# zhvng/open-musiclm

Measured on NVIDIA H100. Metric: coarse-stage training tokens/sec (positions fed to the transformer per optimiser step / step time), higher is better.
Workload: dtype bf16 (fp16 operands for the forward GEMMs on LayerNorm outputs x weights; fp32 accumulate)

## Files before the change

open-musiclm_b200/csrc/gemm_tc.cu:

```cuda
#include "common.cuh"
#include "ptx.cuh"
#include "../../include/omlm_b200.h"
#include <stdlib.h>
#include <algorithm>

namespace omlm {

constexpr int BM = 128;
constexpr int BK = 64;
constexpr int kGemmThreads = 384;

struct EpiParams {
  void* out;
  const float* addend;
  long ldo;
  long ldadd;
  float alpha;
  int out_f32;
  int atomic;
  long split_stride;
  int vec_ok;
  int row_split;
  int row_valid;
  int n_valid;
  const __nv_bfloat16* rs_hn;
  long rs_ldhn;
  const float* rs_gamma;
  const uint8_t* rs_keep;
  float2* rs_part;
  float rs_keep_scale;
  int rs_parts;
};

__device__ __forceinline__ float bf16lo(uint32_t v) { return __uint_as_float(v << 16); }
__device__ __forceinline__ float bf16hi(uint32_t v) { return __uint_as_float(v & 0xffff0000u); }

template <int BN>
struct GemmSmem {
  static constexpr int kABytes = BM * BK * 2;
  static constexpr int kBBytes = BN * BK * 2;
  static constexpr int kStageBytes = kABytes + kBBytes;
  static constexpr int kMaxStages = 8;
};

template <int BN, int A_MN, int B_MN, bool F16, bool RS = false>
__global__ void __launch_bounds__(kGemmThreads, 1)
gemm_bf16_kernel(const __grid_constant__ CUtensorMap tmA, const __grid_constant__ CUtensorMap tmB,
                 const EpiParams ep, const int M, const int N, const int K, const int splits, const int kStages) {
  using S = GemmSmem<BN>;
  extern __shared__ uint8_t smem_raw[];
  uint8_t* smem = smem_raw + ((1024u - (smem_u32(smem_raw) & 1023u)) & 1023u);
  uint64_t* full_bar = reinterpret_cast<uint64_t*>(smem + kStages * S::kStageBytes);
  uint64_t* empty_bar = full_bar + S::kMaxStages;

  const int wg = threadIdx.x >> 7;
  const int lane = threadIdx.x & 31;

  const int m_tiles = (M + BM - 1) / BM;
  const int n_tiles = (N + BN - 1) / BN;
  const int kb_total = (K + BK - 1) / BK;
  const int kb_per_split = (kb_total + splits - 1) / splits;
  const int tiles_total = m_tiles * n_tiles;
  const int work_total = tiles_total * splits;

  if (threadIdx.x == 0) {
    tma_prefetch_desc(&tmA);
    tma_prefetch_desc(&tmB);
    for (int i = 0; i < kStages; ++i) {
      mbar_init(&full_bar[i], 1);
      mbar_init(&empty_bar[i], 2);
    }
    fence_barrier_init();
  }
  __syncthreads();

  if (wg == 0) {
    asm volatile("setmaxnreg.dec.sync.aligned.u32 40;");
    if (threadIdx.x == 0) {
      int stage = 0;
      uint32_t phase = 0;
      for (int w = blockIdx.x; w < work_total; w += gridDim.x) {
        const int split = w / tiles_total;
        const int tile = w - split * tiles_total;
        const int n_blk = tile % n_tiles, m_blk = tile / n_tiles;
        const int kb0 = split * kb_per_split;
        const int kb1 = min(kb_total, kb0 + kb_per_split);
        for (int kb = kb0; kb < kb1; ++kb) {
          mbar_wait(&empty_bar[stage], phase ^ 1);
          uint8_t* sa = smem + stage * S::kStageBytes;
          uint8_t* sb = sa + S::kABytes;
          mbar_expect_tx(&full_bar[stage], S::kStageBytes);
          if (A_MN == 0) {
            tma_load_2d(sa, &tmA, &full_bar[stage], kb * BK, m_blk * BM);
          } else {
#pragma unroll
            for (int c = 0; c < BM / 64; ++c)
              tma_load_2d(sa + c * 8192, &tmA, &full_bar[stage], m_blk * BM + c * 64, kb * BK);
          }
          if (B_MN == 0) {
            tma_load_2d(sb, &tmB, &full_bar[stage], kb * BK, n_blk * BN);
          } else {
#pragma unroll
            for (int c = 0; c < BN / 64; ++c)
              tma_load_2d(sb + c * 8192, &tmB, &full_bar[stage], n_blk * BN + c * 64, kb * BK);
          }
          if (++stage == kStages) { stage = 0; phase ^= 1; }
        }
      }
    }
    return;
  }

  asm volatile("setmaxnreg.inc.sync.aligned.u32 232;");
  const int cw = wg - 1;
  const int wq = (threadIdx.x >> 5) & 3;
  const int qr = lane >> 2, qc = lane & 3;
  const bool leader = (threadIdx.x & 127) == 0;
  int stage = 0;
  uint32_t phase = 0;
  for (int w = blockIdx.x; w < work_total; w += gridDim.x) {
    const int split = w / tiles_total;
    const int tile = w - split * tiles_total;
    const int n_blk = tile % n_tiles, m_blk = tile / n_tiles;
    const int kb0 = split * kb_per_split;
    const int kb1 = min(kb_total, kb0 + kb_per_split);
    float acc[BN / 2];
#pragma unroll
    for (int i = 0; i < BN / 2; ++i) acc[i] = 0.f;
    int prev = -1;
    for (int kb = kb0; kb < kb1; ++kb) {
      mbar_wait(&full_bar[stage], phase);
      const uint32_t sa = smem_u32(smem + stage * S::kStageBytes) + cw * 8192;
      const uint32_t sb = smem_u32(smem + stage * S::kStageBytes + S::kABytes);
      wgmma_fence();
#pragma unroll
      for (int k = 0; k < BK / 16; ++k) {
        const uint64_t ad = A_MN ? make_smem_desc(sa + k * 2048, 8192, 1024) : make_smem_desc(sa + k * 32, 16, 1024);
        const uint64_t bd = B_MN ? make_smem_desc(sb + k * 2048, 8192, 1024) : make_smem_desc(sb + k * 32, 16, 1024);
        const uint32_t accum = (kb > kb0 || k > 0) ? 1u : 0u;
        Wgmma<BN, F16>::template ss<A_MN, B_MN>(acc, ad, bd, accum);
      }
      wgmma_commit();
      wgmma_wait<1>();
      if (prev >= 0 && leader) mbar_arrive(&empty_bar[prev]);
      prev = stage;
      if (++stage == kStages) { stage = 0; phase ^= 1; }
    }
    wgmma_wait<0>();
    wgmma_reg_fence(acc);
    if (prev >= 0 && leader) mbar_arrive(&empty_bar[prev]);

    int row_in[2];
    long orow[2], arow[2];
    bool row_ok[2];
#pragma unroll
    for (int hr = 0; hr < 2; ++hr) {
      int row = m_blk * BM + cw * 64 + wq * 16 + qr + hr * 8;
      row_in[hr] = row;
      row_ok[hr] = row < M;
      if (ep.row_split > 0) {
        const int half = row / ep.row_split, r = row - half * ep.row_split;
        row_ok[hr] = row_ok[hr] && r < ep.row_valid;
        row = half * ep.row_valid + r;
      } else if (ep.row_split < 0) {
        const int w256 = row & 255, ch = ((row >> 8) << 7) + (w256 & 127);
        row_ok[hr] = row_ok[hr] && ch < ep.row_valid;
        row = (w256 >> 7) * ep.row_valid + ch;
      }
      orow[hr] = static_cast<long>(row) * ep.ldo;
      arow[hr] = static_cast<long>(row) * ep.ldadd;
    }
    constexpr int kEpiBatch = RS ? 4 : 8;
    float rs1[2][2] = {{0.f, 0.f}, {0.f, 0.f}}, rs2[2][2] = {{0.f, 0.f}, {0.f, 0.f}};
#pragma unroll
    for (int i0 = 0; i0 < BN / 8; i0 += kEpiBatch) {
      float2 add[2][kEpiBatch], gam[kEpiBatch];
      uint32_t hv[2][kEpiBatch], keep[2][kEpiBatch];
#pragma unroll
      for (int j = 0; j < kEpiBatch; ++j) {
        const int col = n_blk * BN + 8 * (i0 + j) + 2 * qc;
        const bool c0_ok = col < ep.n_valid, c1_ok = col + 1 < ep.n_valid;
        if constexpr (RS) gam[j] = c0_ok ? __ldg(reinterpret_cast<const float2*>(ep.rs_gamma + col)) : make_float2(0.f, 0.f);
#pragma unroll
        for (int hr = 0; hr < 2; ++hr) {
          add[hr][j] = make_float2(0.f, 0.f);
          hv[hr][j] = 0u;
          keep[hr][j] = 0xffu;
          if (!row_ok[hr] || !c0_ok) continue;
          if (!RS && ep.addend != nullptr) {
            const float* ap = ep.addend + arow[hr] + col;
            if (c1_ok && ep.vec_ok) add[hr][j] = *reinterpret_cast<const float2*>(ap);
            else { add[hr][j].x = ap[0]; if (c1_ok) add[hr][j].y = ap[1]; }
          }
          if constexpr (RS) {
            hv[hr][j] = *reinterpret_cast<const uint32_t*>(ep.rs_hn + static_cast<long>(row_in[hr]) * ep.rs_ldhn + col);
            if (ep.rs_keep != nullptr) keep[hr][j] = ep.rs_keep[static_cast<long>(row_in[hr]) * (N >> 3) + (col >> 3)];
          }
        }
      }
#pragma unroll
      for (int j = 0; j < kEpiBatch; ++j) {
        const int i = i0 + j;
        const int col = n_blk * BN + 8 * i + 2 * qc;
        if (col >= ep.n_valid) continue;
        const bool pair = col + 1 < ep.n_valid && ep.vec_ok;
#pragma unroll
        for (int hr = 0; hr < 2; ++hr) {
          if (!row_ok[hr]) continue;
          float v0 = acc[4 * i + 2 * hr] * ep.alpha, v1 = acc[4 * i + 2 * hr + 1] * ep.alpha;
          if constexpr (RS) {
            const uint32_t kb = keep[hr][j];
            const float2 g = gam[j];
            const int hf = (8 * i) / (BN / 2);
            rs1[hr][hf] = fmaf(g.x, ((kb >> (col & 7)) & 1u) ? v0 : 0.f, rs1[hr][hf]);
            rs1[hr][hf] = fmaf(g.y, ((kb >> ((col + 1) & 7)) & 1u) ? v1 : 0.f, rs1[hr][hf]);
            rs2[hr][hf] = fmaf(v0, bf16lo(hv[hr][j]), rs2[hr][hf]);
            rs2[hr][hf] = fmaf(v1, bf16hi(hv[hr][j]), rs2[hr][hf]);
          }
          if (!RS && ep.addend != nullptr) { v0 += add[hr][j].x; v1 += add[hr][j].y; }
          if (ep.atomic) {
            float* op = reinterpret_cast<float*>(ep.out) + orow[hr] + col;
            if (pair) asm volatile("red.global.add.v2.f32 [%0], {%1, %2};" ::"l"(op), "f"(v0), "f"(v1) : "memory");
            else { atomicAdd(op, v0); if (col + 1 < ep.n_valid) atomicAdd(op + 1, v1); }
          } else if (ep.out_f32) {
            float* op = reinterpret_cast<float*>(ep.out) + split * ep.split_stride + orow[hr] + col;
            if (pair) *reinterpret_cast<float2*>(op) = make_float2(v0, v1);
            else { op[0] = v0; if (col + 1 < ep.n_valid) op[1] = v1; }
          } else {
            __nv_bfloat16* op = reinterpret_cast<__nv_bfloat16*>(ep.out) + orow[hr] + col;
            if (pair) *reinterpret_cast<uint32_t*>(op) = pack_bf16x2(v0, v1);
            else { op[0] = __float2bfloat16_rn(v0); if (col + 1 < ep.n_valid) op[1] = __float2bfloat16_rn(v1); }
          }
        }
      }
    }
    if constexpr (RS) {
#pragma unroll
      for (int hr = 0; hr < 2; ++hr)
#pragma unroll
        for (int hf = 0; hf < 2; ++hf) {
          float a1 = rs1[hr][hf], a2 = rs2[hr][hf];
          a1 += __shfl_xor_sync(0xffffffffu, a1, 1); a1 += __shfl_xor_sync(0xffffffffu, a1, 2);
          a2 += __shfl_xor_sync(0xffffffffu, a2, 1); a2 += __shfl_xor_sync(0xffffffffu, a2, 2);
          const int row = m_blk * BM + cw * 64 + wq * 16 + qr + hr * 8;
          if (qc == 0 && row < M) ep.rs_part[static_cast<long>(row) * ep.rs_parts + 2 * n_blk + hf] = make_float2(a1 * ep.rs_keep_scale, a2);
        }
    }
  }
}

constexpr int kMaxDynSmem = 232448;
constexpr int kBarrierBytes = 256;

template <int BN, int A_MN, int B_MN, bool RS = false>
static int launch_gemm(const CUtensorMap& tmA, const CUtensorMap& tmB, const EpiParams& ep, int M, int N, int K, int splits,
                       int max_ctas, int f16, cudaStream_t stream) {
  using S = GemmSmem<BN>;
  auto kern = f16 ? gemm_bf16_kernel<BN, A_MN, B_MN, true, RS> : gemm_bf16_kernel<BN, A_MN, B_MN, false, RS>;
  int stages = (kMaxDynSmem - 1024 - kBarrierBytes) / S::kStageBytes;
  if (stages > 6) stages = 6;
  const int smem_bytes = stages * S::kStageBytes + kBarrierBytes + 1024;
  static bool configured[2] = {false, false};
  if (!configured[f16]) {
    OMLM_CUDA(cudaFuncSetAttribute(kern, cudaFuncAttributeMaxDynamicSharedMemorySize, kMaxDynSmem));
    configured[f16] = true;
  }
  const int m_tiles = (M + BM - 1) / BM, n_tiles = (N + BN - 1) / BN;
  const int work = m_tiles * n_tiles * splits;
  int grid = num_sms();
  if (max_ctas > 0 && max_ctas < grid) grid = max_ctas;
  if (work < grid) grid = work;
  OMLM_KLAUNCH((kern), grid, kGemmThreads, smem_bytes, stream, tmA, tmB, ep, M, N, K, splits, stages);
  OMLM_LAUNCH_CHECK();
  return 0;
}

}

namespace omlm {
struct RowStatArgs { const void* hn; long ldhn; const void* keep_bits; const float* gamma; float keep_scale; float* part; int parts; };
}

static int gemm16_impl(const void* A, int a_f16, int a_mn_major, long lda, const void* B, int b_f16, int b_mn_major,
                       long ldb, int M, int N, int K, void* out, int out_f32, long ldo,
                       const float* addend, long ldadd, float alpha, int splits,
                       int row_split, int row_valid, int n_valid, int block_n, int max_ctas,
                       void* stream_, const omlm::RowStatArgs* rs, long split_stride = 0) {
  using namespace omlm;
  cudaStream_t stream = reinterpret_cast<cudaStream_t>(stream_);
  OMLM_CHECK_ARG(M > 0 && N > 0 && K > 0, "gemm: empty problem %d x %d x %d", M, N, K);
  OMLM_CHECK_ARG(block_n == 128 || block_n == 256, "gemm: block_n must be 128 or 256");
  OMLM_CHECK_ARG(splits >= 1, "gemm: splits must be >= 1");
  OMLM_CHECK_ARG((a_f16 != 0) == (b_f16 != 0), "gemm: both operands must have the same 16-bit format (one wgmma takes one operand format)");
  OMLM_CHECK_ARG(splits == 1 || (out_f32 && addend == nullptr), "gemm: split-K needs fp32 atomic output and no addend");
  OMLM_CHECK_ARG(split_stride == 0 || (out_f32 && addend == nullptr && rs == nullptr), "gemm: partial slices need fp32 output");
  if (n_valid <= 0 || n_valid > N) n_valid = N;
  {
    const int kb_total = (K + BK - 1) / BK;
    if (splits > kb_total) splits = kb_total;
    const int per = (kb_total + splits - 1) / splits;
    splits = (kb_total + per - 1) / per;
  }
  CUtensorMap tmA, tmB;
  int rc;
  if (a_mn_major == 0) rc = make_tmap_bf16_2d(&tmA, A, (uint64_t)K, (uint64_t)M, (uint64_t)lda * 2, 64, BM);
  else                 rc = make_tmap_bf16_2d(&tmA, A, (uint64_t)M, (uint64_t)K, (uint64_t)lda * 2, 64, 64);
  if (rc) return rc;
  if (b_mn_major == 0) rc = make_tmap_bf16_2d(&tmB, B, (uint64_t)K, (uint64_t)N, (uint64_t)ldb * 2, 64, block_n);
  else                 rc = make_tmap_bf16_2d(&tmB, B, (uint64_t)N, (uint64_t)K, (uint64_t)ldb * 2, 64, 64);
  if (rc) return rc;
  EpiParams ep;
  ep.out = out; ep.addend = addend; ep.ldo = ldo; ep.ldadd = ldadd; ep.alpha = alpha;
  ep.out_f32 = out_f32; ep.atomic = (splits > 1 && split_stride == 0) ? 1 : 0; ep.split_stride = split_stride;
  const long esz = out_f32 ? 4 : 2;
  ep.vec_ok = ((ldo * esz) % 16 == 0) && ((reinterpret_cast<uintptr_t>(out) & 15) == 0) &&
              (addend == nullptr || ((ldadd * 4) % 16 == 0 && (reinterpret_cast<uintptr_t>(addend) & 15) == 0));
  ep.row_split = row_split; ep.row_valid = row_valid; ep.n_valid = n_valid;
  ep.rs_hn = nullptr; ep.rs_ldhn = 0; ep.rs_gamma = nullptr; ep.rs_keep = nullptr; ep.rs_part = nullptr; ep.rs_keep_scale = 1.f;
  ep.rs_parts = 0;
  const int f16 = a_f16 ? 1 : 0;
  const int key = (block_n == 256 ? 4 : 0) | (a_mn_major ? 2 : 0) | (b_mn_major ? 1 : 0);
  if (rs != nullptr) {
    OMLM_CHECK_ARG(block_n == 256 && N % 256 == 0 && n_valid == N && !out_f32 && addend == nullptr && splits == 1 && row_split == 0 &&
                   ep.vec_ok && rs->parts == 2 * (N / 256) && rs->ldhn % 8 == 0,
                   "gemm row statistics: needs 256-wide tiles, N %% 256 == 0, a dense bf16 output and parts == N / 128");
    OMLM_CHECK_ARG(key == 5, "gemm row statistics: only the A K-major / B MN-major 256-wide instantiation exists");
    ep.rs_hn = reinterpret_cast<const __nv_bfloat16*>(rs->hn); ep.rs_ldhn = rs->ldhn;
    ep.rs_gamma = rs->gamma; ep.rs_keep = reinterpret_cast<const uint8_t*>(rs->keep_bits);
    ep.rs_part = reinterpret_cast<float2*>(rs->part); ep.rs_keep_scale = rs->keep_scale; ep.rs_parts = rs->parts;
    return launch_gemm<256, 0, 1, true>(tmA, tmB, ep, M, N, K, splits, max_ctas, f16, stream);
  }
  switch (key) {
    case 0: return launch_gemm<128, 0, 0>(tmA, tmB, ep, M, N, K, splits, max_ctas, f16, stream);
    case 1: return launch_gemm<128, 0, 1>(tmA, tmB, ep, M, N, K, splits, max_ctas, f16, stream);
    case 3: return launch_gemm<128, 1, 1>(tmA, tmB, ep, M, N, K, splits, max_ctas, f16, stream);
    case 4: return launch_gemm<256, 0, 0>(tmA, tmB, ep, M, N, K, splits, max_ctas, f16, stream);
    case 5: return launch_gemm<256, 0, 1>(tmA, tmB, ep, M, N, K, splits, max_ctas, f16, stream);
    case 7: return launch_gemm<256, 1, 1>(tmA, tmB, ep, M, N, K, splits, max_ctas, f16, stream);
    default:
      set_last_error("gemm: operand majors (a_mn=%d, b_mn=%d) not instantiated", a_mn_major, b_mn_major);
      return 1;
  }
}

extern "C" int omlm_gemm16(const void* A, int a_f16, int a_mn_major, long lda, const void* B, int b_f16, int b_mn_major,
                           long ldb, int M, int N, int K, void* out, int out_f32, long ldo,
                           const float* addend, long ldadd, float alpha, int splits,
                           int row_split, int row_valid, int n_valid, int block_n, int max_ctas,
                           void* stream_) {
  return gemm16_impl(A, a_f16, a_mn_major, lda, B, b_f16, b_mn_major, ldb, M, N, K, out, out_f32, ldo, addend, ldadd, alpha, splits,
                     row_split, row_valid, n_valid, block_n, max_ctas, stream_, nullptr);
}

namespace omlm {
__global__ void __launch_bounds__(256)
splitk_reduce_kernel(float* __restrict__ out, long ldo, const float* __restrict__ part, long slice, long ldp, int splits,
                     int rows_out, int n_valid) {
  const long total = static_cast<long>(rows_out) * n_valid;
  for (long i = blockIdx.x * static_cast<long>(blockDim.x) + threadIdx.x; i < total; i += static_cast<long>(gridDim.x) * blockDim.x) {
    const long r = i / n_valid, c = i - r * n_valid;
    float v = out[r * ldo + c];
    for (int s = 0; s < splits; ++s) v += part[s * slice + r * ldp + c];
    out[r * ldo + c] = v;
  }
}

static int gemm_rows_out(int M, int row_split, int row_valid) {
  if (row_split > 0) return (M + row_split - 1) / row_split * row_valid;
  if (row_split < 0) return 2 * row_valid;
  return M;
}

static int gemm_splits_effective(int K, int splits) {
  const int kb_total = (K + BK - 1) / BK;
  if (splits > kb_total) splits = kb_total;
  if (splits < 1) splits = 1;
  const int per = (kb_total + splits - 1) / splits;
  return (kb_total + per - 1) / per;
}
}

extern "C" int omlm_gemm16_splitk_det_workspace(int M, int N, int K, int splits, int row_split, int row_valid, int n_valid,
                                                long* part_bytes) {
  using namespace omlm;
  OMLM_CHECK_ARG(M > 0 && N > 0 && K > 0 && splits >= 1 && part_bytes != nullptr, "gemm16_splitk_det_workspace: bad arguments");
  if (n_valid <= 0 || n_valid > N) n_valid = N;
  OMLM_CHECK_ARG(row_split <= 0 || M % row_split == 0, "gemm16_splitk_det: M (%d) must be whole halves of row_split (%d)", M, row_split);
  const int s = gemm_splits_effective(K, splits);
  *part_bytes = s > 1 ? static_cast<long>(s) * gemm_rows_out(M, row_split, row_valid) * ((n_valid + 3) / 4 * 4) * 4 : 0;
  return 0;
}

extern "C" int omlm_gemm16_splitk_det(const void* A, int a_f16, int a_mn_major, long lda, const void* B, int b_f16, int b_mn_major,
                                      long ldb, int M, int N, int K, float* out, long ldo, int splits, int row_split, int row_valid,
                                      int n_valid, int block_n, int max_ctas, float* part_ws, long part_ws_bytes, void* stream_) {
  using namespace omlm;
  OMLM_CHECK_ARG(M > 0 && N > 0 && K > 0 && splits >= 1, "gemm16_splitk_det: empty problem %d x %d x %d", M, N, K);
  if (n_valid <= 0 || n_valid > N) n_valid = N;
  const int s = gemm_splits_effective(K, splits);
  OMLM_CHECK_ARG(row_split <= 0 || M % row_split == 0, "gemm16_splitk_det: M (%d) must be whole halves of row_split (%d)", M, row_split);
  if (s == 1)
    return gemm16_impl(A, a_f16, a_mn_major, lda, B, b_f16, b_mn_major, ldb, M, N, K, out, 1, ldo, out, ldo, 1.f, 1,
                       row_split, row_valid, n_valid, block_n, max_ctas, stream_, nullptr);
  const int rows_out = gemm_rows_out(M, row_split, row_valid);
  const long ldp = (n_valid + 3) / 4 * 4;
  const long slice = static_cast<long>(rows_out) * ldp;
  OMLM_CHECK_ARG(part_ws != nullptr && part_ws_bytes >= s * slice * 4 && (reinterpret_cast<uintptr_t>(part_ws) & 15) == 0,
                 "gemm16_splitk_det: partials need %ld bytes (16-byte aligned), got %ld", s * slice * 4, part_ws_bytes);
  int rc = gemm16_impl(A, a_f16, a_mn_major, lda, B, b_f16, b_mn_major, ldb, M, N, K, part_ws, 1, ldp, nullptr, 0, 1.f, s,
                       row_split, row_valid, n_valid, block_n, max_ctas, stream_, nullptr, slice);
  if (rc) return rc;
  const long total = static_cast<long>(rows_out) * n_valid;
  const int grid = static_cast<int>(std::min<long>((total + 255) / 256, static_cast<long>(num_sms()) * 8));
  OMLM_KLAUNCH((splitk_reduce_kernel), grid, 256, 0, reinterpret_cast<cudaStream_t>(stream_), out, ldo,
               static_cast<const float*>(part_ws), slice, ldp, s, rows_out, n_valid);
  OMLM_LAUNCH_CHECK();
  return 0;
}

extern "C" int omlm_gemm16_rowstat(const void* A, int a_f16, int a_mn_major, long lda, const void* B, int b_f16, int b_mn_major,
                                   long ldb, int M, int N, int K, void* out_bf16, long ldo, const void* hn_bf16, long ldhn,
                                   const void* keep_bits, const float* gamma, float keep_scale, float* part, int parts,
                                   int max_ctas, void* stream_) {
  omlm::RowStatArgs rs{hn_bf16, ldhn, keep_bits, gamma, keep_scale, part, parts};
  return gemm16_impl(A, a_f16, a_mn_major, lda, B, b_f16, b_mn_major, ldb, M, N, K, out_bf16, 0, ldo, nullptr, 0, 1.f, 1,
                     0, 0, N, 256, max_ctas, stream_, &rs);
}

extern "C" int omlm_gemm_bf16(const void* A, int a_mn_major, long lda, const void* B, int b_mn_major,
                              long ldb, int M, int N, int K, void* out, int out_f32, long ldo,
                              const float* addend, long ldadd, float alpha, int splits,
                              int row_split, int row_valid, int n_valid, int block_n, int max_ctas,
                              void* stream_) {
  return omlm_gemm16(A, 0, a_mn_major, lda, B, 0, b_mn_major, ldb, M, N, K, out, out_f32, ldo, addend, ldadd, alpha, splits,
                     row_split, row_valid, n_valid, block_n, max_ctas, stream_);
}
```

open-musiclm_b200/csrc/ptx.cuh:

```cuda
#pragma once
#include <cuda_runtime.h>
#include <cuda_bf16.h>
#include <cuda.h>
#include <stdint.h>

namespace omlm {

__device__ __forceinline__ uint32_t smem_u32(const void* p) {
  return static_cast<uint32_t>(__cvta_generic_to_shared(p));
}
__device__ __forceinline__ uint32_t lane_id() { return threadIdx.x & 31; }

__device__ __forceinline__ bool elect_one() {
  uint32_t pred;
  asm volatile(
      "{\n\t.reg .pred p;\n\t"
      "elect.sync _|p, 0xffffffff;\n\t"
      "selp.u32 %0, 1, 0, p;\n\t}"
      : "=r"(pred));
  return pred != 0;
}

__device__ __forceinline__ void mbar_init(uint64_t* bar, uint32_t count) {
  asm volatile("mbarrier.init.shared::cta.b64 [%0], %1;" ::"r"(smem_u32(bar)), "r"(count));
}
__device__ __forceinline__ void fence_barrier_init() {
  asm volatile("fence.mbarrier_init.release.cluster;" ::: "memory");
}
__device__ __forceinline__ void fence_proxy_async() {
  asm volatile("fence.proxy.async.shared::cta;" ::: "memory");
}
__device__ __forceinline__ void mbar_expect_tx(uint64_t* bar, uint32_t bytes) {
  asm volatile("mbarrier.arrive.expect_tx.shared::cta.b64 _, [%0], %1;" ::"r"(smem_u32(bar)),
               "r"(bytes)
               : "memory");
}
__device__ __forceinline__ void mbar_arrive(uint64_t* bar) {
  asm volatile("mbarrier.arrive.shared::cta.b64 _, [%0];" ::"r"(smem_u32(bar)) : "memory");
}
__device__ __forceinline__ void mbar_wait(uint64_t* bar, uint32_t parity) {
  asm volatile(
      "{\n\t.reg .pred p;\n\t"
      "WAIT_LOOP:\n\t"
      "mbarrier.try_wait.parity.shared::cta.b64 p, [%0], %1;\n\t"
      "@p bra DONE;\n\t"
      "bra WAIT_LOOP;\n\t"
      "DONE:\n\t}"
      ::"r"(smem_u32(bar)), "r"(parity)
      : "memory");
}

__device__ __forceinline__ void tma_prefetch_desc(const CUtensorMap* m) {
  asm volatile("prefetch.tensormap [%0];" ::"l"(reinterpret_cast<uint64_t>(m)) : "memory");
}
__device__ __forceinline__ void tma_load_2d(void* smem_dst, const CUtensorMap* m, uint64_t* bar,
                                            int32_t c0, int32_t c1) {
  asm volatile(
      "cp.async.bulk.tensor.2d.shared::cluster.global.mbarrier::complete_tx::bytes"
      " [%0], [%1, {%3, %4}], [%2];"
      ::"r"(smem_u32(smem_dst)), "l"(reinterpret_cast<uint64_t>(m)), "r"(smem_u32(bar)), "r"(c0),
      "r"(c1)
      : "memory");
}
__device__ __forceinline__ void tma_store_2d(const CUtensorMap* m, const void* smem_src, int32_t c0,
                                             int32_t c1) {
  asm volatile("cp.async.bulk.tensor.2d.global.shared::cta.bulk_group [%0, {%2, %3}], [%1];"
               ::"l"(reinterpret_cast<uint64_t>(m)), "r"(smem_u32(smem_src)), "r"(c0), "r"(c1)
               : "memory");
}
__device__ __forceinline__ void tma_store_3d(const CUtensorMap* m, const void* smem_src, int32_t c0, int32_t c1,
                                             int32_t c2) {
  asm volatile("cp.async.bulk.tensor.3d.global.shared::cta.bulk_group [%0, {%2, %3, %4}], [%1];"
               ::"l"(reinterpret_cast<uint64_t>(m)), "r"(smem_u32(smem_src)), "r"(c0), "r"(c1), "r"(c2)
               : "memory");
}
__device__ __forceinline__ void tma_store_commit() {
  asm volatile("cp.async.bulk.commit_group;" ::: "memory");
}
__device__ __forceinline__ void tma_store_wait_all() {
  asm volatile("cp.async.bulk.wait_group 0;" ::: "memory");
}
template <int N>
__device__ __forceinline__ void tma_store_wait_read() {
  asm volatile("cp.async.bulk.wait_group.read %0;" ::"n"(N) : "memory");
}

__device__ __forceinline__ void wgmma_fence() { asm volatile("wgmma.fence.sync.aligned;" ::: "memory"); }
__device__ __forceinline__ void wgmma_commit() { asm volatile("wgmma.commit_group.sync.aligned;" ::: "memory"); }
template <int N>
__device__ __forceinline__ void wgmma_wait() { asm volatile("wgmma.wait_group.sync.aligned %0;" ::"n"(N) : "memory"); }
template <int R>
__device__ __forceinline__ void wgmma_reg_fence(float (&d)[R]) {
#pragma unroll
  for (int i = 0; i < R; ++i) asm volatile("" : "+f"(d[i])::"memory");
}

__device__ __forceinline__ uint64_t make_smem_desc(uint32_t smem_addr, uint32_t lbo_bytes,
                                                   uint32_t sbo_bytes) {
  uint64_t d = 0;
  d |= static_cast<uint64_t>((smem_addr & 0x3FFFF) >> 4);
  d |= static_cast<uint64_t>((lbo_bytes >> 4) & 0x3FFF) << 16;
  d |= static_cast<uint64_t>((sbo_bytes >> 4) & 0x3FFF) << 32;
  d |= static_cast<uint64_t>(1) << 62;
  return d;
}

template <int N, bool F16> struct Wgmma;
template <> struct Wgmma<64, false> {
  template <int TA, int TB>
  static __device__ __forceinline__ void ss(float (&d)[32], uint64_t a, uint64_t b, uint32_t scale_d) {
    asm volatile(
        "{\n.reg .pred p;\nsetp.ne.b32 p, %34, 0;\n"
        "wgmma.mma_async.sync.aligned.m64n64k16.f32.bf16.bf16 {%0,%1,%2,%3,%4,%5,%6,%7,%8,%9,%10,%11,%12,%13,%14,%15,%16,%17,%18,%19,%20,%21,%22,%23,%24,%25,%26,%27,%28,%29,%30,%31}, %32, %33, p, 1, 1, %35, %36;\n}\n"
        : "+f"(d[0]), "+f"(d[1]), "+f"(d[2]), "+f"(d[3]), "+f"(d[4]), "+f"(d[5]), "+f"(d[6]), "+f"(d[7]), "+f"(d[8]), "+f"(d[9]), "+f"(d[10]), "+f"(d[11]), "+f"(d[12]), "+f"(d[13]), "+f"(d[14]), "+f"(d[15]), "+f"(d[16]), "+f"(d[17]), "+f"(d[18]), "+f"(d[19]), "+f"(d[20]), "+f"(d[21]), "+f"(d[22]), "+f"(d[23]), "+f"(d[24]), "+f"(d[25]), "+f"(d[26]), "+f"(d[27]), "+f"(d[28]), "+f"(d[29]), "+f"(d[30]), "+f"(d[31])
        : "l"(a), "l"(b), "r"(scale_d), "n"(TA), "n"(TB));
  }
  template <int TB>
  static __device__ __forceinline__ void rs(float (&d)[32], const uint32_t (&a)[4], uint64_t b, uint32_t scale_d) {
    asm volatile(
        "{\n.reg .pred p;\nsetp.ne.b32 p, %37, 0;\n"
        "wgmma.mma_async.sync.aligned.m64n64k16.f32.bf16.bf16 {%0,%1,%2,%3,%4,%5,%6,%7,%8,%9,%10,%11,%12,%13,%14,%15,%16,%17,%18,%19,%20,%21,%22,%23,%24,%25,%26,%27,%28,%29,%30,%31}, {%32,%33,%34,%35}, %36, p, 1, 1, %38;\n}\n"
        : "+f"(d[0]), "+f"(d[1]), "+f"(d[2]), "+f"(d[3]), "+f"(d[4]), "+f"(d[5]), "+f"(d[6]), "+f"(d[7]), "+f"(d[8]), "+f"(d[9]), "+f"(d[10]), "+f"(d[11]), "+f"(d[12]), "+f"(d[13]), "+f"(d[14]), "+f"(d[15]), "+f"(d[16]), "+f"(d[17]), "+f"(d[18]), "+f"(d[19]), "+f"(d[20]), "+f"(d[21]), "+f"(d[22]), "+f"(d[23]), "+f"(d[24]), "+f"(d[25]), "+f"(d[26]), "+f"(d[27]), "+f"(d[28]), "+f"(d[29]), "+f"(d[30]), "+f"(d[31])
        : "r"(a[0]), "r"(a[1]), "r"(a[2]), "r"(a[3]), "l"(b), "r"(scale_d), "n"(TB));
  }
};
template <> struct Wgmma<64, true> {
  template <int TA, int TB>
  static __device__ __forceinline__ void ss(float (&d)[32], uint64_t a, uint64_t b, uint32_t scale_d) {
    asm volatile(
        "{\n.reg .pred p;\nsetp.ne.b32 p, %34, 0;\n"
        "wgmma.mma_async.sync.aligned.m64n64k16.f32.f16.f16 {%0,%1,%2,%3,%4,%5,%6,%7,%8,%9,%10,%11,%12,%13,%14,%15,%16,%17,%18,%19,%20,%21,%22,%23,%24,%25,%26,%27,%28,%29,%30,%31}, %32, %33, p, 1, 1, %35, %36;\n}\n"
        : "+f"(d[0]), "+f"(d[1]), "+f"(d[2]), "+f"(d[3]), "+f"(d[4]), "+f"(d[5]), "+f"(d[6]), "+f"(d[7]), "+f"(d[8]), "+f"(d[9]), "+f"(d[10]), "+f"(d[11]), "+f"(d[12]), "+f"(d[13]), "+f"(d[14]), "+f"(d[15]), "+f"(d[16]), "+f"(d[17]), "+f"(d[18]), "+f"(d[19]), "+f"(d[20]), "+f"(d[21]), "+f"(d[22]), "+f"(d[23]), "+f"(d[24]), "+f"(d[25]), "+f"(d[26]), "+f"(d[27]), "+f"(d[28]), "+f"(d[29]), "+f"(d[30]), "+f"(d[31])
        : "l"(a), "l"(b), "r"(scale_d), "n"(TA), "n"(TB));
  }
  template <int TB>
  static __device__ __forceinline__ void rs(float (&d)[32], const uint32_t (&a)[4], uint64_t b, uint32_t scale_d) {
    asm volatile(
        "{\n.reg .pred p;\nsetp.ne.b32 p, %37, 0;\n"
        "wgmma.mma_async.sync.aligned.m64n64k16.f32.f16.f16 {%0,%1,%2,%3,%4,%5,%6,%7,%8,%9,%10,%11,%12,%13,%14,%15,%16,%17,%18,%19,%20,%21,%22,%23,%24,%25,%26,%27,%28,%29,%30,%31}, {%32,%33,%34,%35}, %36, p, 1, 1, %38;\n}\n"
        : "+f"(d[0]), "+f"(d[1]), "+f"(d[2]), "+f"(d[3]), "+f"(d[4]), "+f"(d[5]), "+f"(d[6]), "+f"(d[7]), "+f"(d[8]), "+f"(d[9]), "+f"(d[10]), "+f"(d[11]), "+f"(d[12]), "+f"(d[13]), "+f"(d[14]), "+f"(d[15]), "+f"(d[16]), "+f"(d[17]), "+f"(d[18]), "+f"(d[19]), "+f"(d[20]), "+f"(d[21]), "+f"(d[22]), "+f"(d[23]), "+f"(d[24]), "+f"(d[25]), "+f"(d[26]), "+f"(d[27]), "+f"(d[28]), "+f"(d[29]), "+f"(d[30]), "+f"(d[31])
        : "r"(a[0]), "r"(a[1]), "r"(a[2]), "r"(a[3]), "l"(b), "r"(scale_d), "n"(TB));
  }
};
template <> struct Wgmma<128, false> {
  template <int TA, int TB>
  static __device__ __forceinline__ void ss(float (&d)[64], uint64_t a, uint64_t b, uint32_t scale_d) {
    asm volatile(
        "{\n.reg .pred p;\nsetp.ne.b32 p, %66, 0;\n"
        "wgmma.mma_async.sync.aligned.m64n128k16.f32.bf16.bf16 {%0,%1,%2,%3,%4,%5,%6,%7,%8,%9,%10,%11,%12,%13,%14,%15,%16,%17,%18,%19,%20,%21,%22,%23,%24,%25,%26,%27,%28,%29,%30,%31,%32,%33,%34,%35,%36,%37,%38,%39,%40,%41,%42,%43,%44,%45,%46,%47,%48,%49,%50,%51,%52,%53,%54,%55,%56,%57,%58,%59,%60,%61,%62,%63}, %64, %65, p, 1, 1, %67, %68;\n}\n"
        : "+f"(d[0]), "+f"(d[1]), "+f"(d[2]), "+f"(d[3]), "+f"(d[4]), "+f"(d[5]), "+f"(d[6]), "+f"(d[7]), "+f"(d[8]), "+f"(d[9]), "+f"(d[10]), "+f"(d[11]), "+f"(d[12]), "+f"(d[13]), "+f"(d[14]), "+f"(d[15]), "+f"(d[16]), "+f"(d[17]), "+f"(d[18]), "+f"(d[19]), "+f"(d[20]), "+f"(d[21]), "+f"(d[22]), "+f"(d[23]), "+f"(d[24]), "+f"(d[25]), "+f"(d[26]), "+f"(d[27]), "+f"(d[28]), "+f"(d[29]), "+f"(d[30]), "+f"(d[31]), "+f"(d[32]), "+f"(d[33]), "+f"(d[34]), "+f"(d[35]), "+f"(d[36]), "+f"(d[37]), "+f"(d[38]), "+f"(d[39]), "+f"(d[40]), "+f"(d[41]), "+f"(d[42]), "+f"(d[43]), "+f"(d[44]), "+f"(d[45]), "+f"(d[46]), "+f"(d[47]), "+f"(d[48]), "+f"(d[49]), "+f"(d[50]), "+f"(d[51]), "+f"(d[52]), "+f"(d[53]), "+f"(d[54]), "+f"(d[55]), "+f"(d[56]), "+f"(d[57]), "+f"(d[58]), "+f"(d[59]), "+f"(d[60]), "+f"(d[61]), "+f"(d[62]), "+f"(d[63])
        : "l"(a), "l"(b), "r"(scale_d), "n"(TA), "n"(TB));
  }
};
template <> struct Wgmma<128, true> {
  template <int TA, int TB>
  static __device__ __forceinline__ void ss(float (&d)[64], uint64_t a, uint64_t b, uint32_t scale_d) {
    asm volatile(
        "{\n.reg .pred p;\nsetp.ne.b32 p, %66, 0;\n"
        "wgmma.mma_async.sync.aligned.m64n128k16.f32.f16.f16 {%0,%1,%2,%3,%4,%5,%6,%7,%8,%9,%10,%11,%12,%13,%14,%15,%16,%17,%18,%19,%20,%21,%22,%23,%24,%25,%26,%27,%28,%29,%30,%31,%32,%33,%34,%35,%36,%37,%38,%39,%40,%41,%42,%43,%44,%45,%46,%47,%48,%49,%50,%51,%52,%53,%54,%55,%56,%57,%58,%59,%60,%61,%62,%63}, %64, %65, p, 1, 1, %67, %68;\n}\n"
        : "+f"(d[0]), "+f"(d[1]), "+f"(d[2]), "+f"(d[3]), "+f"(d[4]), "+f"(d[5]), "+f"(d[6]), "+f"(d[7]), "+f"(d[8]), "+f"(d[9]), "+f"(d[10]), "+f"(d[11]), "+f"(d[12]), "+f"(d[13]), "+f"(d[14]), "+f"(d[15]), "+f"(d[16]), "+f"(d[17]), "+f"(d[18]), "+f"(d[19]), "+f"(d[20]), "+f"(d[21]), "+f"(d[22]), "+f"(d[23]), "+f"(d[24]), "+f"(d[25]), "+f"(d[26]), "+f"(d[27]), "+f"(d[28]), "+f"(d[29]), "+f"(d[30]), "+f"(d[31]), "+f"(d[32]), "+f"(d[33]), "+f"(d[34]), "+f"(d[35]), "+f"(d[36]), "+f"(d[37]), "+f"(d[38]), "+f"(d[39]), "+f"(d[40]), "+f"(d[41]), "+f"(d[42]), "+f"(d[43]), "+f"(d[44]), "+f"(d[45]), "+f"(d[46]), "+f"(d[47]), "+f"(d[48]), "+f"(d[49]), "+f"(d[50]), "+f"(d[51]), "+f"(d[52]), "+f"(d[53]), "+f"(d[54]), "+f"(d[55]), "+f"(d[56]), "+f"(d[57]), "+f"(d[58]), "+f"(d[59]), "+f"(d[60]), "+f"(d[61]), "+f"(d[62]), "+f"(d[63])
        : "l"(a), "l"(b), "r"(scale_d), "n"(TA), "n"(TB));
  }
};
template <> struct Wgmma<256, false> {
  template <int TA, int TB>
  static __device__ __forceinline__ void ss(float (&d)[128], uint64_t a, uint64_t b, uint32_t scale_d) {
    asm volatile(
        "{\n.reg .pred p;\nsetp.ne.b32 p, %130, 0;\n"
        "wgmma.mma_async.sync.aligned.m64n256k16.f32.bf16.bf16 {%0,%1,%2,%3,%4,%5,%6,%7,%8,%9,%10,%11,%12,%13,%14,%15,%16,%17,%18,%19,%20,%21,%22,%23,%24,%25,%26,%27,%28,%29,%30,%31,%32,%33,%34,%35,%36,%37,%38,%39,%40,%41,%42,%43,%44,%45,%46,%47,%48,%49,%50,%51,%52,%53,%54,%55,%56,%57,%58,%59,%60,%61,%62,%63,%64,%65,%66,%67,%68,%69,%70,%71,%72,%73,%74,%75,%76,%77,%78,%79,%80,%81,%82,%83,%84,%85,%86,%87,%88,%89,%90,%91,%92,%93,%94,%95,%96,%97,%98,%99,%100,%101,%102,%103,%104,%105,%106,%107,%108,%109,%110,%111,%112,%113,%114,%115,%116,%117,%118,%119,%120,%121,%122,%123,%124,%125,%126,%127}, %128, %129, p, 1, 1, %131, %132;\n}\n"
        : "+f"(d[0]), "+f"(d[1]), "+f"(d[2]), "+f"(d[3]), "+f"(d[4]), "+f"(d[5]), "+f"(d[6]), "+f"(d[7]), "+f"(d[8]), "+f"(d[9]), "+f"(d[10]), "+f"(d[11]), "+f"(d[12]), "+f"(d[13]), "+f"(d[14]), "+f"(d[15]), "+f"(d[16]), "+f"(d[17]), "+f"(d[18]), "+f"(d[19]), "+f"(d[20]), "+f"(d[21]), "+f"(d[22]), "+f"(d[23]), "+f"(d[24]), "+f"(d[25]), "+f"(d[26]), "+f"(d[27]), "+f"(d[28]), "+f"(d[29]), "+f"(d[30]), "+f"(d[31]), "+f"(d[32]), "+f"(d[33]), "+f"(d[34]), "+f"(d[35]), "+f"(d[36]), "+f"(d[37]), "+f"(d[38]), "+f"(d[39]), "+f"(d[40]), "+f"(d[41]), "+f"(d[42]), "+f"(d[43]), "+f"(d[44]), "+f"(d[45]), "+f"(d[46]), "+f"(d[47]), "+f"(d[48]), "+f"(d[49]), "+f"(d[50]), "+f"(d[51]), "+f"(d[52]), "+f"(d[53]), "+f"(d[54]), "+f"(d[55]), "+f"(d[56]), "+f"(d[57]), "+f"(d[58]), "+f"(d[59]), "+f"(d[60]), "+f"(d[61]), "+f"(d[62]), "+f"(d[63]), "+f"(d[64]), "+f"(d[65]), "+f"(d[66]), "+f"(d[67]), "+f"(d[68]), "+f"(d[69]), "+f"(d[70]), "+f"(d[71]), "+f"(d[72]), "+f"(d[73]), "+f"(d[74]), "+f"(d[75]), "+f"(d[76]), "+f"(d[77]), "+f"(d[78]), "+f"(d[79]), "+f"(d[80]), "+f"(d[81]), "+f"(d[82]), "+f"(d[83]), "+f"(d[84]), "+f"(d[85]), "+f"(d[86]), "+f"(d[87]), "+f"(d[88]), "+f"(d[89]), "+f"(d[90]), "+f"(d[91]), "+f"(d[92]), "+f"(d[93]), "+f"(d[94]), "+f"(d[95]), "+f"(d[96]), "+f"(d[97]), "+f"(d[98]), "+f"(d[99]), "+f"(d[100]), "+f"(d[101]), "+f"(d[102]), "+f"(d[103]), "+f"(d[104]), "+f"(d[105]), "+f"(d[106]), "+f"(d[107]), "+f"(d[108]), "+f"(d[109]), "+f"(d[110]), "+f"(d[111]), "+f"(d[112]), "+f"(d[113]), "+f"(d[114]), "+f"(d[115]), "+f"(d[116]), "+f"(d[117]), "+f"(d[118]), "+f"(d[119]), "+f"(d[120]), "+f"(d[121]), "+f"(d[122]), "+f"(d[123]), "+f"(d[124]), "+f"(d[125]), "+f"(d[126]), "+f"(d[127])
        : "l"(a), "l"(b), "r"(scale_d), "n"(TA), "n"(TB));
  }
};
template <> struct Wgmma<256, true> {
  template <int TA, int TB>
  static __device__ __forceinline__ void ss(float (&d)[128], uint64_t a, uint64_t b, uint32_t scale_d) {
    asm volatile(
        "{\n.reg .pred p;\nsetp.ne.b32 p, %130, 0;\n"
        "wgmma.mma_async.sync.aligned.m64n256k16.f32.f16.f16 {%0,%1,%2,%3,%4,%5,%6,%7,%8,%9,%10,%11,%12,%13,%14,%15,%16,%17,%18,%19,%20,%21,%22,%23,%24,%25,%26,%27,%28,%29,%30,%31,%32,%33,%34,%35,%36,%37,%38,%39,%40,%41,%42,%43,%44,%45,%46,%47,%48,%49,%50,%51,%52,%53,%54,%55,%56,%57,%58,%59,%60,%61,%62,%63,%64,%65,%66,%67,%68,%69,%70,%71,%72,%73,%74,%75,%76,%77,%78,%79,%80,%81,%82,%83,%84,%85,%86,%87,%88,%89,%90,%91,%92,%93,%94,%95,%96,%97,%98,%99,%100,%101,%102,%103,%104,%105,%106,%107,%108,%109,%110,%111,%112,%113,%114,%115,%116,%117,%118,%119,%120,%121,%122,%123,%124,%125,%126,%127}, %128, %129, p, 1, 1, %131, %132;\n}\n"
        : "+f"(d[0]), "+f"(d[1]), "+f"(d[2]), "+f"(d[3]), "+f"(d[4]), "+f"(d[5]), "+f"(d[6]), "+f"(d[7]), "+f"(d[8]), "+f"(d[9]), "+f"(d[10]), "+f"(d[11]), "+f"(d[12]), "+f"(d[13]), "+f"(d[14]), "+f"(d[15]), "+f"(d[16]), "+f"(d[17]), "+f"(d[18]), "+f"(d[19]), "+f"(d[20]), "+f"(d[21]), "+f"(d[22]), "+f"(d[23]), "+f"(d[24]), "+f"(d[25]), "+f"(d[26]), "+f"(d[27]), "+f"(d[28]), "+f"(d[29]), "+f"(d[30]), "+f"(d[31]), "+f"(d[32]), "+f"(d[33]), "+f"(d[34]), "+f"(d[35]), "+f"(d[36]), "+f"(d[37]), "+f"(d[38]), "+f"(d[39]), "+f"(d[40]), "+f"(d[41]), "+f"(d[42]), "+f"(d[43]), "+f"(d[44]), "+f"(d[45]), "+f"(d[46]), "+f"(d[47]), "+f"(d[48]), "+f"(d[49]), "+f"(d[50]), "+f"(d[51]), "+f"(d[52]), "+f"(d[53]), "+f"(d[54]), "+f"(d[55]), "+f"(d[56]), "+f"(d[57]), "+f"(d[58]), "+f"(d[59]), "+f"(d[60]), "+f"(d[61]), "+f"(d[62]), "+f"(d[63]), "+f"(d[64]), "+f"(d[65]), "+f"(d[66]), "+f"(d[67]), "+f"(d[68]), "+f"(d[69]), "+f"(d[70]), "+f"(d[71]), "+f"(d[72]), "+f"(d[73]), "+f"(d[74]), "+f"(d[75]), "+f"(d[76]), "+f"(d[77]), "+f"(d[78]), "+f"(d[79]), "+f"(d[80]), "+f"(d[81]), "+f"(d[82]), "+f"(d[83]), "+f"(d[84]), "+f"(d[85]), "+f"(d[86]), "+f"(d[87]), "+f"(d[88]), "+f"(d[89]), "+f"(d[90]), "+f"(d[91]), "+f"(d[92]), "+f"(d[93]), "+f"(d[94]), "+f"(d[95]), "+f"(d[96]), "+f"(d[97]), "+f"(d[98]), "+f"(d[99]), "+f"(d[100]), "+f"(d[101]), "+f"(d[102]), "+f"(d[103]), "+f"(d[104]), "+f"(d[105]), "+f"(d[106]), "+f"(d[107]), "+f"(d[108]), "+f"(d[109]), "+f"(d[110]), "+f"(d[111]), "+f"(d[112]), "+f"(d[113]), "+f"(d[114]), "+f"(d[115]), "+f"(d[116]), "+f"(d[117]), "+f"(d[118]), "+f"(d[119]), "+f"(d[120]), "+f"(d[121]), "+f"(d[122]), "+f"(d[123]), "+f"(d[124]), "+f"(d[125]), "+f"(d[126]), "+f"(d[127])
        : "l"(a), "l"(b), "r"(scale_d), "n"(TA), "n"(TB));
  }
};

}
```

Measured before the change: 584,400.

## Stage bf16 GEMM epilogue through shared memory and write it with TMA stores

For plain bf16 outputs (no split-K, addend, row remap or row stats), each consumer warpgroup packs its accumulators into a swizzled shared-memory staging buffer and issues 2D TMA bulk stores, replacing scattered per-thread global writes. The goal is to cut epilogue store cost and overlap it with the next tile's mainloop. In exchange, staging buffers reserve extra shared memory, which may reduce pipeline stages for large BN, and named barriers are added. The TMA store relies on the tensor map clipping columns past n_valid and rows past M.

```diff
diff --git a/open-musiclm_b200/csrc/gemm_tc.cu b/open-musiclm_b200/csrc/gemm_tc.cu
--- a/open-musiclm_b200/csrc/gemm_tc.cu
+++ b/open-musiclm_b200/csrc/gemm_tc.cu
@@ -30,6 +30,7 @@
   float2* rs_part;
   float rs_keep_scale;
   int rs_parts;
+  int tma_out;
 };
 
 __device__ __forceinline__ float bf16lo(uint32_t v) { return __uint_as_float(v << 16); }
@@ -42,11 +43,13 @@
   static constexpr int kStageBytes = kABytes + kBBytes;
   static constexpr int kMaxStages = 8;
 };
+constexpr int kStgBoxBytes = 64 * 64 * 2;
+constexpr int kStgBytes = 2 * kStgBoxBytes;
 
 template <int BN, int A_MN, int B_MN, bool F16, bool RS = false>
 __global__ void __launch_bounds__(kGemmThreads, 1)
 gemm_bf16_kernel(const __grid_constant__ CUtensorMap tmA, const __grid_constant__ CUtensorMap tmB,
-                 const EpiParams ep, const int M, const int N, const int K, const int splits, const int kStages) {
+                 const __grid_constant__ CUtensorMap tmC, const EpiParams ep, const int M, const int N, const int K, const int splits, const int kStages) {
   using S = GemmSmem<BN>;
   extern __shared__ uint8_t smem_raw[];
   uint8_t* smem = smem_raw + ((1024u - (smem_u32(smem_raw) & 1023u)) & 1023u);
@@ -66,6 +69,7 @@
   if (threadIdx.x == 0) {
     tma_prefetch_desc(&tmA);
     tma_prefetch_desc(&tmB);
+    if (ep.tma_out) tma_prefetch_desc(&tmC);
     for (int i = 0; i < kStages; ++i) {
       mbar_init(&full_bar[i], 1);
       mbar_init(&empty_bar[i], 2);
@@ -150,6 +154,34 @@
     wgmma_reg_fence(acc);
     if (prev >= 0 && leader) mbar_arrive(&empty_bar[prev]);
 
+    if (!RS && ep.tma_out) {
+      uint8_t* stg = smem + kStages * S::kStageBytes + 1024 + cw * kStgBytes;
+#pragma unroll
+      for (int half = 0; half < BN / 128; ++half) {
+        if (leader) tma_store_wait_read<0>();
+        named_bar_sync(1 + cw, 128);
+#pragma unroll
+        for (int i = 0; i < 16; ++i) {
+          const int ig = half * 16 + i;
+#pragma unroll
+          for (int hr = 0; hr < 2; ++hr) {
+            const int r = wq * 16 + qr + hr * 8;
+            *reinterpret_cast<uint32_t*>(stg + (i >> 3) * kStgBoxBytes + r * 128 + (((i & 7) ^ qr) << 4) + qc * 4) =
+                pack_bf16x2(acc[4 * ig + 2 * hr] * ep.alpha, acc[4 * ig + 2 * hr + 1] * ep.alpha);
+          }
+        }
+        fence_proxy_async();
+        named_bar_sync(1 + cw, 128);
+        if (leader) {
+          const int col = n_blk * BN + half * 128, row = m_blk * BM + cw * 64;
+          tma_store_2d(&tmC, stg, col, row);
+          tma_store_2d(&tmC, stg + kStgBoxBytes, col + 64, row);
+          tma_store_commit();
+        }
+      }
+      continue;
+    }
+
     int row_in[2];
     long orow[2], arow[2];
     bool row_ok[2];
@@ -247,19 +279,20 @@
         }
     }
   }
+  if (!RS && ep.tma_out && leader) tma_store_wait_all();
 }
 
 constexpr int kMaxDynSmem = 232448;
-constexpr int kBarrierBytes = 256;
+constexpr int kBarrierBytes = 1024;
 
 template <int BN, int A_MN, int B_MN, bool RS = false>
-static int launch_gemm(const CUtensorMap& tmA, const CUtensorMap& tmB, const EpiParams& ep, int M, int N, int K, int splits,
+static int launch_gemm(const CUtensorMap& tmA, const CUtensorMap& tmB, const CUtensorMap& tmC, const EpiParams& ep, int M, int N, int K, int splits,
                        int max_ctas, int f16, cudaStream_t stream) {
   using S = GemmSmem<BN>;
   auto kern = f16 ? gemm_bf16_kernel<BN, A_MN, B_MN, true, RS> : gemm_bf16_kernel<BN, A_MN, B_MN, false, RS>;
-  int stages = (kMaxDynSmem - 1024 - kBarrierBytes) / S::kStageBytes;
+  int stages = (kMaxDynSmem - 1024 - kBarrierBytes - 2 * kStgBytes) / S::kStageBytes;
   if (stages > 6) stages = 6;
-  const int smem_bytes = stages * S::kStageBytes + kBarrierBytes + 1024;
+  const int smem_bytes = stages * S::kStageBytes + kBarrierBytes + 2 * kStgBytes + 1024;
   static bool configured[2] = {false, false};
   if (!configured[f16]) {
     OMLM_CUDA(cudaFuncSetAttribute(kern, cudaFuncAttributeMaxDynamicSharedMemorySize, kMaxDynSmem));
@@ -270,7 +303,7 @@
   int grid = num_sms();
   if (max_ctas > 0 && max_ctas < grid) grid = max_ctas;
   if (work < grid) grid = work;
-  OMLM_KLAUNCH((kern), grid, kGemmThreads, smem_bytes, stream, tmA, tmB, ep, M, N, K, splits, stages);
+  OMLM_KLAUNCH((kern), grid, kGemmThreads, smem_bytes, stream, tmA, tmB, tmC, ep, M, N, K, splits, stages);
   OMLM_LAUNCH_CHECK();
   return 0;
 }
@@ -318,6 +351,13 @@
   ep.row_split = row_split; ep.row_valid = row_valid; ep.n_valid = n_valid;
   ep.rs_hn = nullptr; ep.rs_ldhn = 0; ep.rs_gamma = nullptr; ep.rs_keep = nullptr; ep.rs_part = nullptr; ep.rs_keep_scale = 1.f;
   ep.rs_parts = 0;
+  ep.tma_out = (rs == nullptr && !out_f32 && addend == nullptr && row_split == 0 && splits == 1 &&
+                (reinterpret_cast<uintptr_t>(out) & 15) == 0 && (ldo * 2) % 16 == 0) ? 1 : 0;
+  CUtensorMap tmC = tmA;
+  if (ep.tma_out) {
+    rc = make_tmap_bf16_2d(&tmC, out, (uint64_t)n_valid, (uint64_t)M, (uint64_t)ldo * 2, 64, 64);
+    if (rc) return rc;
+  }
   const int f16 = a_f16 ? 1 : 0;
   const int key = (block_n == 256 ? 4 : 0) | (a_mn_major ? 2 : 0) | (b_mn_major ? 1 : 0);
   if (rs != nullptr) {
@@ -328,15 +368,15 @@
     ep.rs_hn = reinterpret_cast<const __nv_bfloat16*>(rs->hn); ep.rs_ldhn = rs->ldhn;
     ep.rs_gamma = rs->gamma; ep.rs_keep = reinterpret_cast<const uint8_t*>(rs->keep_bits);
     ep.rs_part = reinterpret_cast<float2*>(rs->part); ep.rs_keep_scale = rs->keep_scale; ep.rs_parts = rs->parts;
-    return launch_gemm<256, 0, 1, true>(tmA, tmB, ep, M, N, K, splits, max_ctas, f16, stream);
+    return launch_gemm<256, 0, 1, true>(tmA, tmB, tmC, ep, M, N, K, splits, max_ctas, f16, stream);
   }
   switch (key) {
-    case 0: return launch_gemm<128, 0, 0>(tmA, tmB, ep, M, N, K, splits, max_ctas, f16, stream);
-    case 1: return launch_gemm<128, 0, 1>(tmA, tmB, ep, M, N, K, splits, max_ctas, f16, stream);
-    case 3: return launch_gemm<128, 1, 1>(tmA, tmB, ep, M, N, K, splits, max_ctas, f16, stream);
-    case 4: return launch_gemm<256, 0, 0>(tmA, tmB, ep, M, N, K, splits, max_ctas, f16, stream);
-    case 5: return launch_gemm<256, 0, 1>(tmA, tmB, ep, M, N, K, splits, max_ctas, f16, stream);
-    case 7: return launch_gemm<256, 1, 1>(tmA, tmB, ep, M, N, K, splits, max_ctas, f16, stream);
+    case 0: return launch_gemm<128, 0, 0>(tmA, tmB, tmC, ep, M, N, K, splits, max_ctas, f16, stream);
+    case 1: return launch_gemm<128, 0, 1>(tmA, tmB, tmC, ep, M, N, K, splits, max_ctas, f16, stream);
+    case 3: return launch_gemm<128, 1, 1>(tmA, tmB, tmC, ep, M, N, K, splits, max_ctas, f16, stream);
+    case 4: return launch_gemm<256, 0, 0>(tmA, tmB, tmC, ep, M, N, K, splits, max_ctas, f16, stream);
+    case 5: return launch_gemm<256, 0, 1>(tmA, tmB, tmC, ep, M, N, K, splits, max_ctas, f16, stream);
+    case 7: return launch_gemm<256, 1, 1>(tmA, tmB, tmC, ep, M, N, K, splits, max_ctas, f16, stream);
     default:
       set_last_error("gemm: operand majors (a_mn=%d, b_mn=%d) not instantiated", a_mn_major, b_mn_major);
       return 1;
diff --git a/open-musiclm_b200/csrc/ptx.cuh b/open-musiclm_b200/csrc/ptx.cuh
--- a/open-musiclm_b200/csrc/ptx.cuh
+++ b/open-musiclm_b200/csrc/ptx.cuh
@@ -48,6 +48,10 @@
       "DONE:\n\t}"
       ::"r"(smem_u32(bar)), "r"(parity)
       : "memory");
+}
+
+__device__ __forceinline__ void named_bar_sync(int id, int threads) {
+  asm volatile("bar.sync %0, %1;" ::"r"(id), "r"(threads) : "memory");
 }
 
 __device__ __forceinline__ void tma_prefetch_desc(const CUtensorMap* m) {
```

Result: faster. 590,700, median of 6 (+1.1%).
